# jiwoon-ahn/irn

Hardware: AMD Instinct MI355X
Metric: images/sec for CAM+random-walk label gen, VOC12 512^2 (random-walk label generation stage) (higher is better)
Workload: dtype f32

## Files before the change

irn_amd/csrc/label.hip:

```cpp
#include "kernels.hpp"
#include "thres_hist.hpp"

#pragma clang fp contract(off)

namespace irn {

struct LabelJob {
    const float *rw;
    const int64_t *keys;
    uint8_t *labels;
    int32_t *argmax;
    float *rw_up;
    unsigned *max_slot;
    int c, h, w, oh, ow;
    const uint8_t *gt;
};

namespace {

__device__ __forceinline__ unsigned enc_ordered(float f) {
    const unsigned b = __float_as_uint(f);
    return (b & 0x80000000u) ? ~b : (b | 0x80000000u);
}
__device__ __forceinline__ float dec_ordered(unsigned u) {
    return __uint_as_float((u & 0x80000000u) ? (u & 0x7fffffffu) : ~u);
}

struct Taps {
    int i0, i1;
    float l0, l1;
};

__device__ __forceinline__ Taps taps_x4(int dst, int n_in) {
    float src = ((float)dst + 0.5f) * 0.25f;
    src = src - 0.5f;
    src = src < 0.f ? 0.f : src;
    Taps t;
    t.i0 = min((int)src, n_in - 1);
    t.i1 = min(t.i0 + 1, n_in - 1);
    t.l1 = src - (float)t.i0;
    t.l0 = 1.0f - t.l1;
    return t;
}

__device__ __forceinline__ float bilerp_vals(float v00, float v01, float v10, float v11, const Taps &ty, const Taps &tx) {
    const float p01 = v01 * tx.l1, p11 = v11 * tx.l1;
    const float top = __builtin_fmaf(v00, tx.l0, p01);
    const float bot = __builtin_fmaf(v10, tx.l0, p11);
    const float pb = ty.l1 * bot;
    return __builtin_fmaf(ty.l0, top, pb);
}

__device__ __forceinline__ float bilerp(const float *__restrict__ plane, int w, const Taps &ty, const Taps &tx) {
    return bilerp_vals(plane[ty.i0 * w + tx.i0], plane[ty.i0 * w + tx.i1], plane[ty.i1 * w + tx.i0], plane[ty.i1 * w + tx.i1], ty, tx);
}

__device__ __forceinline__ void block_max_to_slot(float m, unsigned *slot) {
    for (int s = 32; s > 0; s >>= 1) m = fmaxf(m, __shfl_xor(m, s));
    __shared__ float wmax[4];
    if ((threadIdx.x & 63) == 0) wmax[threadIdx.x >> 6] = m;
    __syncthreads();
    if (threadIdx.x == 0) {
        m = fmaxf(fmaxf(wmax[0], wmax[1]), fmaxf(wmax[2], wmax[3]));
        if (m > -INFINITY) atomicMax(slot, enc_ordered(m));
    }
}

__device__ __forceinline__ int cell_lo(int k) { return k == 0 ? 0 : 4 * k + 2; }

template <int PASS>
__global__ __launch_bounds__(256) void upsample_max_kernel(const LabelJob *__restrict__ jobs) {
    const LabelJob J = jobs[blockIdx.y];
    const unsigned plane_px = (unsigned)(J.h * J.w), cells = (unsigned)J.c * plane_px;
    const float lower = PASS == 2 ? dec_ordered(*J.max_slot) : 0.f;
    float m = -INFINITY;
    for (unsigned i = blockIdx.x * 256 + threadIdx.x; i < cells; i += gridDim.x * 256) {
        const int c = (int)(i / plane_px);
        const int r = (int)(i - (unsigned)c * plane_px);
        const int k = (int)((unsigned)r / (unsigned)J.w), l = r - k * J.w;
        const int y0 = cell_lo(k), x0 = cell_lo(l);
        if (y0 >= J.oh || x0 >= J.ow) continue;
        const float *plane = J.rw + (long)c * J.h * J.w;
        if (PASS == 1) {
            m = fmaxf(m, bilerp(plane, J.w, taps_x4(y0, J.h), taps_x4(x0, J.w)));
        } else {
            const int k1 = min(k + 1, J.h - 1), l1 = min(l + 1, J.w - 1);
            const float u = fmaxf(fmaxf(plane[k * J.w + l], plane[k * J.w + l1]), fmaxf(plane[k1 * J.w + l], plane[k1 * J.w + l1]));
            if (u + fabsf(u) * 1e-6f + 1e-37f < lower) continue;
            const int y1 = min(k == J.h - 1 ? 4 * J.h - 1 : 4 * k + 5, J.oh - 1);
            const int x1 = min(l == J.w - 1 ? 4 * J.w - 1 : 4 * l + 5, J.ow - 1);
            for (int oy = y0; oy <= y1; ++oy) {
                const Taps ty = taps_x4(oy, J.h);
                for (int ox = x0; ox <= x1; ++ox) m = fmaxf(m, bilerp(plane, J.w, ty, taps_x4(ox, J.w)));
            }
        }
    }
    block_max_to_slot(m, J.max_slot);
}

struct Group {
    int oy, ox, nq;
    unsigned o;
    Taps ty, tx[4];
};

__device__ __forceinline__ Group group_of(const LabelJob &J, unsigned g, unsigned gw) {
    Group G;
    G.oy = (int)(g / gw), G.ox = (int)(g - (unsigned)G.oy * gw) * 4;
    G.nq = min(4, J.ow - G.ox);
    G.o = (unsigned)G.oy * (unsigned)J.ow + (unsigned)G.ox;
    G.ty = taps_x4(G.oy, J.h);
#pragma unroll
    for (int q = 0; q < 4; ++q) G.tx[q] = taps_x4(min(G.ox + q, J.ow - 1), J.w);
    return G;
}

__device__ __forceinline__ void group_scores(const LabelJob &J, const Group &G, int c, float gmax, float (&v)[4]) {
    const Taps &ty = G.ty, *tx = G.tx;
    const float *r0 = J.rw + (long)c * J.h * J.w + ty.i0 * J.w, *r1 = J.rw + (long)c * J.h * J.w + ty.i1 * J.w;
    const float a00 = r0[tx[0].i0], a01 = r0[tx[0].i1], a10 = r1[tx[0].i0], a11 = r1[tx[0].i1];
    const float b00 = r0[tx[2].i0], b01 = r0[tx[2].i1], b10 = r1[tx[2].i0], b11 = r1[tx[2].i1];
    v[0] = bilerp_vals(a00, a01, a10, a11, ty, tx[0]) / gmax;
    v[1] = bilerp_vals(a00, a01, a10, a11, ty, tx[1]) / gmax;
    v[2] = bilerp_vals(b00, b01, b10, b11, ty, tx[2]) / gmax;
    v[3] = bilerp_vals(b00, b01, b10, b11, ty, tx[3]) / gmax;
}

__global__ __launch_bounds__(256) void label_argmax_kernel(const LabelJob *__restrict__ jobs, float bg) {
    const LabelJob J = jobs[blockIdx.y];
    const unsigned gw = (unsigned)(J.ow + 3) >> 2, groups = gw * (unsigned)J.oh;
    const unsigned npx = (unsigned)J.oh * (unsigned)J.ow;
    const float gmax = dec_ordered(*J.max_slot);
    for (unsigned g = blockIdx.x * 256 + threadIdx.x; g < groups; g += gridDim.x * 256) {
        const Group G = group_of(J, g, gw);
        float best[4] = {bg, bg, bg, bg};
        int idx[4] = {0, 0, 0, 0};
        for (int c = 0; c < J.c; ++c) {
            float v[4];
            group_scores(J, G, c, gmax, v);
            if (J.rw_up) {
                float *dst = J.rw_up + (long)c * npx + G.o;
                if (G.nq == 4 && ((uintptr_t)dst & 15) == 0) *reinterpret_cast<float4 *>(dst) = make_float4(v[0], v[1], v[2], v[3]);
                else
                    for (int q = 0; q < G.nq; ++q) dst[q] = v[q];
            }
#pragma unroll
            for (int q = 0; q < 4; ++q)
                if (v[q] > best[q] || (v[q] != v[q] && best[q] == best[q])) {
                    best[q] = v[q];
                    idx[q] = c + 1;
                }
        }
        if (J.argmax) {
            int32_t *dst = J.argmax + G.o;
            if (G.nq == 4 && ((uintptr_t)dst & 15) == 0) *reinterpret_cast<int4 *>(dst) = make_int4(idx[0], idx[1], idx[2], idx[3]);
            else
                for (int q = 0; q < G.nq; ++q) dst[q] = idx[q];
        }
        if (J.labels) {
            uint8_t lab[4];
#pragma unroll
            for (int q = 0; q < 4; ++q) lab[q] = idx[q] == 0 ? (uint8_t)0 : (uint8_t)(J.keys[idx[q] - 1] + 1);
            uint8_t *dst = J.labels + G.o;
            if (G.nq == 4 && ((uintptr_t)dst & 3) == 0)
                *reinterpret_cast<uint32_t *>(dst) = (uint32_t)lab[0] | ((uint32_t)lab[1] << 8) | ((uint32_t)lab[2] << 16) | ((uint32_t)lab[3] << 24);
            else
                for (int q = 0; q < G.nq; ++q) dst[q] = lab[q];
        }
    }
}

constexpr int kSweepGroups = 4;
constexpr int kSweepChunk = 256 * kSweepGroups;
constexpr int kSweepCap = 15360;
static_assert(thist::kThreads == 256, "thres_hist.hpp counts with blocks of this size");

__global__ __launch_bounds__(256) void label_sweep_kernel(const LabelJob *__restrict__ jobs, const float *__restrict__ thres,
                                                          int t, int cap, int64_t *__restrict__ hist, int64_t *__restrict__ bad) {
    extern __shared__ __attribute__((aligned(16))) uint32_t sweep_lds[];
    uint32_t *bins = sweep_lds;
    float *th = reinterpret_cast<float *>(sweep_lds + cap);
    int *col = reinterpret_cast<int *>(th + IRN_EVAL_MAX_THRES);
    uint32_t *nbad = reinterpret_cast<uint32_t *>(col + thist::kMaxKeys);
    const LabelJob J = jobs[blockIdx.y];
    uint32_t local_bad = thist::stage(thres, t, J.keys, J.c, blockIdx.x == 0 && blockIdx.y == 0, th, col, nbad);

    const unsigned gw = (unsigned)(J.ow + 3) >> 2, groups = gw * (unsigned)J.oh;
    const unsigned chunks = (groups + kSweepChunk - 1) / kSweepChunk;
    const uint32_t nbins = (uint32_t)(t + 1) * thist::kRows * (uint32_t)J.c;
    const float gmax = dec_ordered(*J.max_slot);
    for (unsigned chunk = blockIdx.x; chunk < chunks; chunk += gridDim.x) {
        uint32_t bin[4 * kSweepGroups];
#pragma unroll
        for (int i = 0; i < kSweepGroups; ++i) {
#pragma unroll
            for (int q = 0; q < 4; ++q) bin[4 * i + q] = thist::kSkip;
            const unsigned g = chunk * kSweepChunk + (unsigned)i * 256 + threadIdx.x;
            if (g >= groups) continue;
            const Group G = group_of(J, g, gw);
            float m[4] = {0.f, 0.f, 0.f, 0.f};
            int cs[4] = {0, 0, 0, 0}, nanc[4] = {-1, -1, -1, -1};
            for (int c = 0; c < J.c; ++c) {
                float v[4];
                group_scores(J, G, c, gmax, v);
#pragma unroll
                for (int q = 0; q < 4; ++q) {
                    if (c == 0 || v[q] > m[q]) {
                        m[q] = v[q];
                        cs[q] = c;
                    }
                    if (v[q] != v[q] && nanc[q] < 0) nanc[q] = c;
                }
            }
            const uint8_t *gp = J.gt + G.o;
            uint8_t gv[4] = {0, 0, 0, 0};
            if (G.nq == 4 && ((uintptr_t)gp & 3) == 0) {
                const uint32_t u = *reinterpret_cast<const uint32_t *>(gp);
                gv[0] = (uint8_t)u; gv[1] = (uint8_t)(u >> 8); gv[2] = (uint8_t)(u >> 16); gv[3] = (uint8_t)(u >> 24);
            } else {
                for (int q = 0; q < G.nq; ++q) gv[q] = gp[q];
            }
#pragma unroll
            for (int q = 0; q < 4; ++q) {
                if (q >= G.nq) continue;
                const int row = thist::gt_row(gv[q]);
                if (row < 0) {
                    ++local_bad;
                    continue;
                }
                const int lo = thist::count_below(th, t, m[q]);
                const int j = nanc[q] >= 0 ? t : lo, cq = nanc[q] >= 0 ? nanc[q] : cs[q];
                bin[4 * i + q] = thist::bin_of(j, row, cq, J.c);
            }
        }
        local_bad += thist::count(bin, bins, (uint32_t)cap, nbins, J.c, col, t, hist);
    }
    thist::flush_bad(local_bad, nbad, bad);
}

constexpr int kMaxScales = 8;
struct MergeArgs {
    const float *src[kMaxScales];
    int hs[kMaxScales], ws[kMaxScales];
    int n_scales, n_cls, k;
    const int64_t *keys;
    float *lo, *hi;
    int lh, lw, uh, uw, H, W;
    unsigned *max_slots;
};

__device__ __forceinline__ Taps taps_resize(int dst, int n_in, int n_out) {
    const float scale = (float)n_in / (float)n_out;
    float src = scale * ((float)dst + 0.5f);
    src = src - 0.5f;
    src = src < 0.f ? 0.f : src;
    Taps t;
    t.i0 = min((int)src, n_in - 1);
    t.i1 = min(t.i0 + 1, n_in - 1);
    t.l1 = src - (float)t.i0;
    t.l0 = 1.0f - t.l1;
    return t;
}

__global__ __launch_bounds__(256) void cam_merge_sum_kernel(const MergeArgs A) {
    const int kk = blockIdx.y;
    const bool is_hi = blockIdx.z == 1;
    const int oh = is_hi ? A.H : A.lh, ow = is_hi ? A.W : A.lw;
    const int th = is_hi ? A.uh : A.lh, tw = is_hi ? A.uw : A.lw;
    float *out = (is_hi ? A.hi : A.lo) + (long)kk * oh * ow;
    const int cls = (int)A.keys[kk];
    float m = -INFINITY;
    for (long o = (long)blockIdx.x * 256 + threadIdx.x; o < (long)oh * ow; o += (long)gridDim.x * 256) {
        const int oy = (int)(o / ow), ox = (int)(o - (long)oy * ow);
        float acc = 0.f;
        for (int s = 0; s < A.n_scales; ++s) {
            const Taps ty = taps_resize(oy, A.hs[s], th), tx = taps_resize(ox, A.ws[s], tw);
            acc = acc + bilerp(A.src[s] + (long)cls * A.hs[s] * A.ws[s], A.ws[s], ty, tx);
        }
        out[o] = acc;
        m = fmaxf(m, acc);
    }
    block_max_to_slot(m, A.max_slots + (is_hi ? A.k : 0) + kk);
}

__global__ __launch_bounds__(256) void cam_merge_norm_kernel(const MergeArgs A) {
    const int kk = blockIdx.y;
    const bool is_hi = blockIdx.z == 1;
    const long n = is_hi ? (long)A.H * A.W : (long)A.lh * A.lw;
    float *out = (is_hi ? A.hi : A.lo) + (long)kk * n;
    const float den = dec_ordered(A.max_slots[(is_hi ? A.k : 0) + kk]) + 1e-5f;
    for (long o = (long)blockIdx.x * 256 + threadIdx.x; o < n; o += (long)gridDim.x * 256) out[o] = out[o] / den;
}

struct LabelBatch {
    std::vector<LabelJob> jobs;
    LabelJob *dev = nullptr;
    long max_px = 0, max_cells = 0;
    int max_c = 0;
};

int label_jobs(const char *who, int n_images, const float *const *rw_dev, const int32_t *c, const int32_t *h, const int32_t *w,
               const int32_t *out_h, const int32_t *out_w, const int64_t *const *keys_dev, uint8_t *const *labels_dev,
               int32_t *const *argmax_dev, float *const *rw_up_dev, const uint8_t *const *gt_dev, void *scratch_dev, LabelBatch &B) {
    B.jobs.resize(n_images);
    for (int i = 0; i < n_images; ++i) {
        if (!rw_dev[i] || c[i] < 1 || h[i] < 1 || w[i] < 1 || out_h[i] < 1 || out_w[i] < 1 || out_h[i] > 4 * h[i] || out_w[i] > 4 * w[i])
            return fail(IRN_ERR_ARG, "%s: image %d: bad sizes (c=%d %dx%d -> %dx%d)", who, i, c[i], h[i], w[i], out_h[i], out_w[i]);
        const LabelJob J = {rw_dev[i], keys_dev ? keys_dev[i] : nullptr, labels_dev ? labels_dev[i] : nullptr,
                            argmax_dev ? argmax_dev[i] : nullptr, rw_up_dev ? rw_up_dev[i] : nullptr, (unsigned *)scratch_dev + i,
                            c[i], h[i], w[i], out_h[i], out_w[i], gt_dev ? gt_dev[i] : nullptr};
        if (J.labels && !J.keys) return fail(IRN_ERR_ARG, "%s: image %d: labels requested without keys", who, i);
        B.jobs[i] = J;
        B.max_px = std::max(B.max_px, (long)out_h[i] * out_w[i]);
        B.max_cells = std::max(B.max_cells, (long)c[i] * h[i] * w[i]);
        B.max_c = std::max(B.max_c, c[i]);
    }
    if (B.max_px >= (1L << 31) || B.max_cells >= (1L << 31)) return fail(IRN_ERR_ARG, "%s: image too large (32-bit pixel indices)", who);
    return IRN_OK;
}

int launch_max_passes(LabelBatch &B, void *scratch_dev, hipStream_t stream) {
    const int n_images = (int)B.jobs.size();
    int rc = scratch_upload(B.jobs.data(), sizeof(LabelJob) * n_images, (void **)&B.dev, stream);
    if (rc) return rc;
    IRN_HIP_TRY(hipMemsetAsync(scratch_dev, 0, sizeof(unsigned) * n_images, stream));
    const long per_image = std::max<long>(1, 4096 / n_images);
    const int bc = (int)std::min<long>((B.max_cells + 255) / 256, per_image);
    hipLaunchKernelGGL(upsample_max_kernel<1>, dim3(bc, n_images), dim3(256), 0, stream, B.dev);
    IRN_LAUNCH_CHECK("upsample_max_kernel<1>");
    hipLaunchKernelGGL(upsample_max_kernel<2>, dim3(bc, n_images), dim3(256), 0, stream, B.dev);
    IRN_LAUNCH_CHECK("upsample_max_kernel<2>");
    return IRN_OK;
}

}
}

using namespace irn;

extern "C" int irn_label_epilogue(int n_images, const float *const *rw_dev, const int32_t *c, const int32_t *h,
                                  const int32_t *w, const int32_t *out_h, const int32_t *out_w, float bg_thres,
                                  const int64_t *const *keys_dev, uint8_t *const *labels_dev,
                                  int32_t *const *argmax_dev, float *const *rw_up_dev, void *scratch_dev,
                                  void *stream_) {
    hipStream_t stream = (hipStream_t)stream_;
    if (n_images < 1 || !rw_dev || !c || !h || !w || !out_h || !out_w || !scratch_dev)
        return fail(IRN_ERR_ARG, "irn_label_epilogue: bad argument");
    LabelBatch B;
    int rc = label_jobs("irn_label_epilogue", n_images, rw_dev, c, h, w, out_h, out_w, keys_dev, labels_dev, argmax_dev, rw_up_dev,
                        nullptr, scratch_dev, B);
    if (rc) return rc;
    rc = launch_max_passes(B, scratch_dev, stream);
    if (rc) return rc;
    const int bx = (int)std::min<long>((B.max_px / 4 + 255) / 256 + 1, 512);
    hipLaunchKernelGGL(label_argmax_kernel, dim3(bx, n_images), dim3(256), 0, stream, B.dev, bg_thres);
    IRN_LAUNCH_CHECK("label_argmax_kernel");
    return scratch_release(stream);
}

extern "C" int irn_label_sweep_confusion(int n_images, const float *const *rw_dev, const int32_t *c, const int32_t *h,
                                         const int32_t *w, const int32_t *out_h, const int32_t *out_w,
                                         const int64_t *const *keys_dev, const uint8_t *const *gt_dev,
                                         const float *thres_dev, int t, int64_t *hist_dev, int64_t *bad_dev,
                                         void *scratch_dev, void *stream_) {
    hipStream_t stream = (hipStream_t)stream_;
    if (n_images < 1 || n_images > 65535 || !rw_dev || !c || !h || !w || !out_h || !out_w || !keys_dev || !gt_dev || !thres_dev ||
        !hist_dev || !bad_dev || !scratch_dev || t < 1 || t > IRN_EVAL_MAX_THRES)
        return fail(IRN_ERR_ARG, "irn_label_sweep_confusion: bad argument (n_images=%d, t=%d; 1 <= t <= %d)", n_images, t,
                    IRN_EVAL_MAX_THRES);
    LabelBatch B;
    int rc = label_jobs("irn_label_sweep_confusion", n_images, rw_dev, c, h, w, out_h, out_w, keys_dev, nullptr, nullptr, nullptr,
                        gt_dev, scratch_dev, B);
    if (rc) return rc;
    for (int i = 0; i < n_images; ++i)
        if (c[i] > thist::kMaxKeys || !keys_dev[i] || !gt_dev[i])
            return fail(IRN_ERR_ARG, "irn_label_sweep_confusion: image %d: c=%d (at most %d), keys and ground truth are required", i,
                        c[i], thist::kMaxKeys);
    rc = launch_max_passes(B, scratch_dev, stream);
    if (rc) return rc;
    const long nbins = (long)(t + 1) * thist::kRows * B.max_c;
    const int cap = (int)std::min<long>((nbins + 3) / 4 * 4, kSweepCap);
    const size_t lds = sizeof(uint32_t) * cap + sizeof(float) * IRN_EVAL_MAX_THRES + sizeof(int) * thist::kMaxKeys + sizeof(uint32_t);
    const int bx = (int)std::min<long>(((B.max_px + 3) / 4 + kSweepChunk - 1) / kSweepChunk + 1, 128);
    hipLaunchKernelGGL(label_sweep_kernel, dim3(bx, n_images), dim3(256), lds, stream, B.dev, thres_dev, t, cap, hist_dev,
                       bad_dev);
    IRN_LAUNCH_CHECK("label_sweep_kernel");
    return scratch_release(stream);
}

extern "C" int irn_cam_merge(int n_scales, const float *const *src_dev, const int32_t *hs, const int32_t *ws, int n_classes,
                             const int64_t *keys_dev, int n_keys, int out_h, int out_w, float *cam_dev,
                             float *high_res_dev, void *scratch_dev, void *stream_) {
    hipStream_t stream = (hipStream_t)stream_;
    if (n_scales < 1 || n_scales > kMaxScales || !src_dev || !hs || !ws || n_classes < 1 || !keys_dev || n_keys < 1 ||
        out_h < 1 || out_w < 1 || !cam_dev || !high_res_dev || !scratch_dev)
        return fail(IRN_ERR_ARG, "irn_cam_merge: bad argument (1..%d scales, >= 1 key)", kMaxScales);
    MergeArgs A;
    for (int s = 0; s < n_scales; ++s) {
        if (!src_dev[s] || hs[s] < 1 || ws[s] < 1) return fail(IRN_ERR_ARG, "irn_cam_merge: scale %d: bad input", s);
        A.src[s] = src_dev[s];
        A.hs[s] = hs[s];
        A.ws[s] = ws[s];
    }
    A.n_scales = n_scales;
    A.n_cls = n_classes;
    A.k = n_keys;
    A.keys = keys_dev;
    A.lo = cam_dev;
    A.hi = high_res_dev;
    A.H = out_h;
    A.W = out_w;
    A.lh = (out_h - 1) / 4 + 1;
    A.lw = (out_w - 1) / 4 + 1;
    A.uh = ((out_h - 1) / 16 + 1) * 16;
    A.uw = ((out_w - 1) / 16 + 1) * 16;
    A.max_slots = (unsigned *)scratch_dev;
    IRN_HIP_TRY(hipMemsetAsync(scratch_dev, 0, sizeof(unsigned) * 2 * n_keys, stream));
    const int bx = (int)std::min<long>(((long)out_h * out_w + 255) / 256, 256);
    hipLaunchKernelGGL(cam_merge_sum_kernel, dim3(bx, n_keys, 2), dim3(256), 0, stream, A);
    IRN_LAUNCH_CHECK("cam_merge_sum_kernel");
    hipLaunchKernelGGL(cam_merge_norm_kernel, dim3(bx, n_keys, 2), dim3(256), 0, stream, A);
    IRN_LAUNCH_CHECK("cam_merge_norm_kernel");
    return IRN_OK;
}
```

Measured before the change: 19640.

## Process four output rows per thread sharing source taps in label argmax kernel

Each argmax thread now handles a block of up to four output rows that fall within one source-row pair, loading the six source values once per class and reusing them for all rows. The grid becomes one group per thread, with no grid-stride loop, and is sized from the per-image group count. Label lookup goes through a shared-memory LUT of keys instead of per-pixel global loads. In exchange each thread uses more registers, and the grid size now scales with image size rather than being capped.

```diff
diff --git a/irn_amd/csrc/label.hip b/irn_amd/csrc/label.hip
--- a/irn_amd/csrc/label.hip
+++ b/irn_amd/csrc/label.hip
@@ -98,74 +98,136 @@
     block_max_to_slot(m, J.max_slot);
 }
 
+constexpr int kBlockRows = 4;
+
+template <int R>
+__host__ __device__ __forceinline__ unsigned row_groups(int oh) {
+    static_assert(R == 1 || R == 4, "one row, or the rows of one source-row pair");
+    return R == 1 ? (unsigned)oh : (unsigned)(oh + 5) >> 2;
+}
+
+template <int R>
 struct Group {
-    int oy, ox, nq;
+    int oy, ox, nr, nq;
     unsigned o;
-    Taps ty, tx[4];
+    int c0, c1, c2;
+    bool b_from_c0;
+    Taps ty[R], tx[4];
 };
 
-__device__ __forceinline__ Group group_of(const LabelJob &J, unsigned g, unsigned gw) {
-    Group G;
-    G.oy = (int)(g / gw), G.ox = (int)(g - (unsigned)G.oy * gw) * 4;
+template <int R>
+__device__ __forceinline__ Group<R> group_of(const LabelJob &J, unsigned g, unsigned gw) {
+    Group<R> G;
+    const int r = (int)(g / gw);
+    G.ox = (int)(g - (unsigned)r * gw) * 4;
+    G.oy = R == 1 || r == 0 ? r : 4 * r - 2;
+    G.nr = R == 1 ? 1 : min(r == 0 ? 2 : 4, J.oh - G.oy);
     G.nq = min(4, J.ow - G.ox);
     G.o = (unsigned)G.oy * (unsigned)J.ow + (unsigned)G.ox;
-    G.ty = taps_x4(G.oy, J.h);
+#pragma unroll
+    for (int i = 0; i < R; ++i) G.ty[i] = taps_x4(G.oy + min(i, G.nr - 1), J.h);
 #pragma unroll
     for (int q = 0; q < 4; ++q) G.tx[q] = taps_x4(min(G.ox + q, J.ow - 1), J.w);
+    G.c0 = G.tx[0].i0, G.c1 = G.tx[0].i1, G.c2 = G.tx[2].i1;
+    G.b_from_c0 = G.tx[2].i0 == G.tx[0].i0;
     return G;
 }
 
-__device__ __forceinline__ void group_scores(const LabelJob &J, const Group &G, int c, float gmax, float (&v)[4]) {
-    const Taps &ty = G.ty, *tx = G.tx;
-    const float *r0 = J.rw + (long)c * J.h * J.w + ty.i0 * J.w, *r1 = J.rw + (long)c * J.h * J.w + ty.i1 * J.w;
-    const float a00 = r0[tx[0].i0], a01 = r0[tx[0].i1], a10 = r1[tx[0].i0], a11 = r1[tx[0].i1];
-    const float b00 = r0[tx[2].i0], b01 = r0[tx[2].i1], b10 = r1[tx[2].i0], b11 = r1[tx[2].i1];
-    v[0] = bilerp_vals(a00, a01, a10, a11, ty, tx[0]) / gmax;
-    v[1] = bilerp_vals(a00, a01, a10, a11, ty, tx[1]) / gmax;
-    v[2] = bilerp_vals(b00, b01, b10, b11, ty, tx[2]) / gmax;
-    v[3] = bilerp_vals(b00, b01, b10, b11, ty, tx[3]) / gmax;
-}
+template <int R>
+__device__ __forceinline__ void group_scores(const LabelJob &J, const Group<R> &G, int c, float gmax, float (&v)[R][4]) {
+    const Taps *tx = G.tx;
+    const float *r0 = J.rw + (long)c * J.h * J.w + G.ty[0].i0 * J.w, *r1 = J.rw + (long)c * J.h * J.w + G.ty[0].i1 * J.w;
+    const float a00 = r0[G.c0], a01 = r0[G.c1], b01 = r0[G.c2], a10 = r1[G.c0], a11 = r1[G.c1], b11 = r1[G.c2];
+    const float b00 = G.b_from_c0 ? a00 : a01, b10 = G.b_from_c0 ? a10 : a11;
+#pragma unroll
+    for (int i = 0; i < R; ++i) {
+        const Taps &ty = G.ty[i];
+        v[i][0] = bilerp_vals(a00, a01, a10, a11, ty, tx[0]) / gmax;
+        v[i][1] = bilerp_vals(a00, a01, a10, a11, ty, tx[1]) / gmax;
+        v[i][2] = bilerp_vals(b00, b01, b10, b11, ty, tx[2]) / gmax;
+        v[i][3] = bilerp_vals(b00, b01, b10, b11, ty, tx[3]) / gmax;
+    }
+}
+
+constexpr int kLutSize = 256;
 
 __global__ __launch_bounds__(256) void label_argmax_kernel(const LabelJob *__restrict__ jobs, float bg) {
+    constexpr int R = kBlockRows;
+    __shared__ uint8_t lut[kLutSize];
     const LabelJob J = jobs[blockIdx.y];
-    const unsigned gw = (unsigned)(J.ow + 3) >> 2, groups = gw * (unsigned)J.oh;
+    const unsigned gw = (unsigned)(J.ow + 3) >> 2, groups = gw * row_groups<R>(J.oh);
+    if (blockIdx.x * 256 >= groups) return;
+    const bool use_lut = J.labels && J.c < kLutSize;
+    if (use_lut) {
+        if ((int)threadIdx.x <= J.c) lut[threadIdx.x] = threadIdx.x == 0 ? (uint8_t)0 : (uint8_t)(J.keys[threadIdx.x - 1] + 1);
+        __syncthreads();
+    }
+    const unsigned g = blockIdx.x * 256 + threadIdx.x;
+    if (g >= groups) return;
     const unsigned npx = (unsigned)J.oh * (unsigned)J.ow;
     const float gmax = dec_ordered(*J.max_slot);
-    for (unsigned g = blockIdx.x * 256 + threadIdx.x; g < groups; g += gridDim.x * 256) {
-        const Group G = group_of(J, g, gw);
-        float best[4] = {bg, bg, bg, bg};
-        int idx[4] = {0, 0, 0, 0};
-        for (int c = 0; c < J.c; ++c) {
-            float v[4];
-            group_scores(J, G, c, gmax, v);
-            if (J.rw_up) {
-                float *dst = J.rw_up + (long)c * npx + G.o;
-                if (G.nq == 4 && ((uintptr_t)dst & 15) == 0) *reinterpret_cast<float4 *>(dst) = make_float4(v[0], v[1], v[2], v[3]);
+    const Group<R> G = group_of<R>(J, g, gw);
+    float best[R][4];
+    int idx[R][4];
+#pragma unroll
+    for (int i = 0; i < R; ++i)
+#pragma unroll
+        for (int q = 0; q < 4; ++q) best[i][q] = bg, idx[i][q] = 0;
+    for (int c = 0; c < J.c; ++c) {
+        float v[R][4];
+        group_scores<R>(J, G, c, gmax, v);
+        if (J.rw_up) {
+#pragma unroll
+            for (int i = 0; i < R; ++i) {
+                if (i >= G.nr) continue;
+                float *dst = J.rw_up + (long)c * npx + G.o + (unsigned)i * (unsigned)J.ow;
+                if (G.nq == 4 && ((uintptr_t)dst & 15) == 0) *reinterpret_cast<float4 *>(dst) = make_float4(v[i][0], v[i][1], v[i][2], v[i][3]);
                 else
-                    for (int q = 0; q < G.nq; ++q) dst[q] = v[q];
-            }
+                    for (int q = 0; q < G.nq; ++q) dst[q] = v[i][q];
+            }
+        }
+#pragma unroll
+        for (int i = 0; i < R; ++i)
 #pragma unroll
             for (int q = 0; q < 4; ++q)
-                if (v[q] > best[q] || (v[q] != v[q] && best[q] == best[q])) {
-                    best[q] = v[q];
-                    idx[q] = c + 1;
+                if (!(v[i][q] <= best[i][q]) && best[i][q] == best[i][q]) {
+                    best[i][q] = v[i][q];
+                    idx[i][q] = c + 1;
                 }
-        }
-        if (J.argmax) {
-            int32_t *dst = J.argmax + G.o;
-            if (G.nq == 4 && ((uintptr_t)dst & 15) == 0) *reinterpret_cast<int4 *>(dst) = make_int4(idx[0], idx[1], idx[2], idx[3]);
+    }
+    if (J.argmax) {
+#pragma unroll
+        for (int i = 0; i < R; ++i) {
+            if (i >= G.nr) continue;
+            int32_t *dst = J.argmax + G.o + (unsigned)i * (unsigned)J.ow;
+            if (G.nq == 4 && ((uintptr_t)dst & 15) == 0) *reinterpret_cast<int4 *>(dst) = make_int4(idx[i][0], idx[i][1], idx[i][2], idx[i][3]);
             else
-                for (int q = 0; q < G.nq; ++q) dst[q] = idx[q];
-        }
-        if (J.labels) {
-            uint8_t lab[4];
-#pragma unroll
-            for (int q = 0; q < 4; ++q) lab[q] = idx[q] == 0 ? (uint8_t)0 : (uint8_t)(J.keys[idx[q] - 1] + 1);
-            uint8_t *dst = J.labels + G.o;
-            if (G.nq == 4 && ((uintptr_t)dst & 3) == 0)
-                *reinterpret_cast<uint32_t *>(dst) = (uint32_t)lab[0] | ((uint32_t)lab[1] << 8) | ((uint32_t)lab[2] << 16) | ((uint32_t)lab[3] << 24);
+                for (int q = 0; q < G.nq; ++q) dst[q] = idx[i][q];
+        }
+    }
+    if (J.labels) {
+        uint32_t lab[R];
+        if (use_lut) {
+#pragma unroll
+            for (int i = 0; i < R; ++i)
+                lab[i] = (uint32_t)lut[idx[i][0]] | ((uint32_t)lut[idx[i][1]] << 8) | ((uint32_t)lut[idx[i][2]] << 16) |
+                         ((uint32_t)lut[idx[i][3]] << 24);
+        } else {
+#pragma unroll
+            for (int i = 0; i < R; ++i) {
+                lab[i] = 0;
+#pragma unroll
+                for (int q = 0; q < 4; ++q)
+                    lab[i] |= (uint32_t)(idx[i][q] == 0 ? (uint8_t)0 : (uint8_t)(J.keys[idx[i][q] - 1] + 1)) << (8 * q);
+            }
+        }
+#pragma unroll
+        for (int i = 0; i < R; ++i) {
+            if (i >= G.nr) continue;
+            uint8_t *dst = J.labels + G.o + (unsigned)i * (unsigned)J.ow;
+            if (G.nq == 4 && ((uintptr_t)dst & 3) == 0) *reinterpret_cast<uint32_t *>(dst) = lab[i];
             else
-                for (int q = 0; q < G.nq; ++q) dst[q] = lab[q];
+                for (int q = 0; q < G.nq; ++q) dst[q] = (uint8_t)(lab[i] >> (8 * q));
         }
     }
 }
@@ -197,19 +259,19 @@
             for (int q = 0; q < 4; ++q) bin[4 * i + q] = thist::kSkip;
             const unsigned g = chunk * kSweepChunk + (unsigned)i * 256 + threadIdx.x;
             if (g >= groups) continue;
-            const Group G = group_of(J, g, gw);
+            const Group<1> G = group_of<1>(J, g, gw);
             float m[4] = {0.f, 0.f, 0.f, 0.f};
             int cs[4] = {0, 0, 0, 0}, nanc[4] = {-1, -1, -1, -1};
             for (int c = 0; c < J.c; ++c) {
-                float v[4];
-                group_scores(J, G, c, gmax, v);
+                float v[1][4];
+                group_scores<1>(J, G, c, gmax, v);
 #pragma unroll
                 for (int q = 0; q < 4; ++q) {
-                    if (c == 0 || v[q] > m[q]) {
-                        m[q] = v[q];
+                    if (c == 0 || v[0][q] > m[q]) {
+                        m[q] = v[0][q];
                         cs[q] = c;
                     }
-                    if (v[q] != v[q] && nanc[q] < 0) nanc[q] = c;
+                    if (v[0][q] != v[0][q] && nanc[q] < 0) nanc[q] = c;
                 }
             }
             const uint8_t *gp = J.gt + G.o;
@@ -352,7 +414,9 @@
     if (rc) return rc;
     rc = launch_max_passes(B, scratch_dev, stream);
     if (rc) return rc;
-    const int bx = (int)std::min<long>((B.max_px / 4 + 255) / 256 + 1, 512);
+    long max_groups = 1;
+    for (const LabelJob &J : B.jobs) max_groups = std::max(max_groups, (long)((J.ow + 3) >> 2) * row_groups<kBlockRows>(J.oh));
+    const int bx = (int)((max_groups + 255) / 256);
     hipLaunchKernelGGL(label_argmax_kernel, dim3(bx, n_images), dim3(256), 0, stream, B.dev, bg_thres);
     IRN_LAUNCH_CHECK("label_argmax_kernel");
     return scratch_release(stream);
```

After: 19730, median of 6. Within noise of the previous version (+0.5%).
